# nk4517/gaussian-splatting-skysphere

Hardware: AMD Instinct MI355X
Metric: train iters/sec (fwd+bwd) + render Mpix/s @1080p, 1M Gaussians SH=3 (higher is better)
Workload: dtype f32; 1 GPU; C3: 1M Gaussians SH3 1920x1080, 16x16 tiles; gaussians=1000000, sh_degree=3, width=1920, height=1080, render_exp2=hardware v_exp_f32, parallelism=view-parallel dp1

## Files before the change

gaussian-splatting-skysphere_amd/csrc/gs_forward.hip:

```cpp
#include "gs_internal.h"

namespace gs {


template <int DEG>
__device__ __forceinline__ void sh_to_rgb(const float* __restrict__ sh, const float* __restrict__ rest, int M, float x,
                                          float y, float z, float* rgb, uint32_t& clamped) {
  constexpr int K = (DEG + 1) * (DEG + 1);
  float s[K * 3];
  if (rest) {
    const F3 d = *reinterpret_cast<const F3*>(sh);
    s[0] = d.a, s[1] = d.b, s[2] = d.c;
    const F3* r3 = reinterpret_cast<const F3*>(rest);
#pragma unroll
    for (int j = 0; j < K - 1; j++) {
      const F3 t = r3[j];
      s[3 + 3 * j] = t.a, s[4 + 3 * j] = t.b, s[5 + 3 * j] = t.c;
    }
  } else if (((M * 3) & 3) == 0) {
    const float4* s4 = reinterpret_cast<const float4*>(sh);
#pragma unroll
    for (int v = 0; v < (K * 3 + 3) / 4; v++) {
      float4 q = s4[v];
      if (4 * v + 0 < K * 3) s[4 * v + 0] = q.x;
// ... 124 lines not shown
    area += (uint32_t)__shfl_xor((int)area, d, 64);
    vis += (uint32_t)__shfl_xor((int)vis, d, 64);
  }
  if ((threadIdx.x & 63) == 0) {
    s_sum[threadIdx.x >> 6] = area;
    s_vis[threadIdx.x >> 6] = vis | (cm ? 0x80000000u : 0u);
  }
  lds_barrier();
  if (threadIdx.x == 0) {
    const uint32_t tot = s_sum[0] + s_sum[1] + s_sum[2] + s_sum[3];
    const uint32_t v4 = s_vis[0] | s_vis[1] | s_vis[2] | s_vis[3];
    const uint32_t nv = (s_vis[0] & 0x7FFFFFFFu) + (s_vis[1] & 0x7FFFFFFFu) + (s_vis[2] & 0x7FFFFFFFu) +
                        (s_vis[3] & 0x7FFFFFFFu);
    store_wg_totals(wg, b, nv, tot, (v4 >> 31) != 0);
  }
}

template <int DEG>
__global__ __launch_bounds__(256) void k_preprocess(GaussianArgs g, CameraArgs c, int* __restrict__ radii,
                                                    float4* __restrict__ splat, float4* __restrict__ binrec,
                                                    uint32_t* __restrict__ depth_key,
                                                    uint32_t* __restrict__ tiles, uint8_t* __restrict__ clamped,
                                                    WgTotals* __restrict__ wg) {
  const int b = (int)blockIdx.x + g.blk0, i = b * 256 + (int)threadIdx.x;
  uint32_t area = 0, dbits = 0;
  bool culled = false;
  if (i < g.P) {
    area = preprocess_one<DEG>(i, g, c, radii, splat, binrec, dbits, tiles, clamped, culled);
    depth_key[i] = area ? dbits : DEPTH_DROP;
  }
  workgroup_totals(area, culled, wg, (uint32_t)b);
}

template <int DEG>
__global__ __launch_bounds__(256) void k_preprocess_split(
    GaussianArgs g, CameraArgs c, int* __restrict__ radii, float4* __restrict__ splat, float4* __restrict__ binrec,
    uint32_t* __restrict__ depth_key, uint32_t* __restrict__ tiles, uint8_t* __restrict__ clamped,
    WgTotals* __restrict__ wg) {
  const int b = (int)blockIdx.x + g.blk0, i = b * 256 + (int)threadIdx.x;
  uint32_t area = 0, dbits = 0;
  bool culled = false;
  if (i < g.P) {
    area = preprocess_one<DEG, true>(i, g, c, radii, splat, binrec, dbits, tiles, clamped, culled);
    depth_key[i] = area ? dbits : DEPTH_DROP;
  }
  workgroup_totals(area, culled, wg, (uint32_t)b);
}

template <class Launch>
static void launch_row_chunks(const GaussianArgs& g, hipStream_t st, Launch&& launch) {
  const int nb = (g.P + 255) / 256;
  RowWait w[GS_MAX_ROW_WAITS];
  const int n = take_row_waits(w, GS_MAX_ROW_WAITS);
  int b0 = 0;
  for (int k = 0; k < n && b0 < nb; k++) {
    if (w[k].ev && !stream_wait(st, w[k].ev)) return;
    const int b1 = w[k].hi >= g.P ? nb : w[k].hi / 256;
    if (b1 > b0) {
      GaussianArgs gc = g;
      gc.blk0 = b0;
      launch(gc, dim3(b1 - b0));
      b0 = b1;
    }
  }
  if (b0 < nb) {
    GaussianArgs gc = g;
    gc.blk0 = b0;
    launch(gc, dim3(nb - b0));
  }
}

void fwd_preprocess(const GaussianArgs& g0, const CameraArgs& c, int* radii, const GeomPtrs& geo, hipStream_t st) {
  launch_row_chunks(g0, st, [&](const GaussianArgs& g, dim3 grid) { fwd_preprocess_grid(g, c, radii, geo, st, grid); });
}

void fwd_preprocess_grid(const GaussianArgs& g, const CameraArgs& c, int* radii, const GeomPtrs& geo, hipStream_t st,
                         dim3 grid) {
  const dim3 block(256);
  if (g.colors) {
    GS_LAUNCH("preprocess", k_preprocess<-1>, grid, block, 0, st, g, c, radii, geo.splat, geo.binrec, geo.keys_a, geo.tiles,
              geo.clamped, geo.wg_tot);
    return;
  }
  if (g.shs_rest) {
#define GS_PRE_SPLIT(D)                                                                                        \
  GS_LAUNCH("preprocess", (k_preprocess_split<D>), grid, block, 0, st, g, c, radii, geo.splat, geo.binrec, \
            geo.keys_a, geo.tiles, geo.clamped, geo.wg_tot)
    switch (g.D) {
      case 0: GS_PRE_SPLIT(0); break;
      case 1: GS_PRE_SPLIT(1); break;
      case 2: GS_PRE_SPLIT(2); break;
      default: GS_PRE_SPLIT(3); break;
    }
#undef GS_PRE_SPLIT
    return;
  }
  switch (g.D) {
    case 0:
      GS_LAUNCH("preprocess", k_preprocess<0>, grid, block, 0, st, g, c, radii, geo.splat, geo.binrec, geo.keys_a, geo.tiles,
                geo.clamped, geo.wg_tot);
      break;
    case 1:
      GS_LAUNCH("preprocess", k_preprocess<1>, grid, block, 0, st, g, c, radii, geo.splat, geo.binrec, geo.keys_a, geo.tiles,
                geo.clamped, geo.wg_tot);
      break;
    case 2:
      GS_LAUNCH("preprocess", k_preprocess<2>, grid, block, 0, st, g, c, radii, geo.splat, geo.binrec, geo.keys_a, geo.tiles,
                geo.clamped, geo.wg_tot);
      break;
    default:
      GS_LAUNCH("preprocess", k_preprocess<3>, grid, block, 0, st, g, c, radii, geo.splat, geo.binrec, geo.keys_a, geo.tiles,
                geo.clamped, geo.wg_tot);
      break;
  }
}

template <int DEG>
__global__ __launch_bounds__(256) void k_preprocess_views(GaussianArgs g, PreViews pv) {
  const int b = (int)blockIdx.x + g.blk0, i = b * 256 + (int)threadIdx.x;
  for (int v = 0; v < pv.K; v++) {
    const GeomPtrs& geo = pv.geo[v];
    uint32_t area = 0, dbits = 0;
    bool culled = false;
    if (i < g.P) {
      area = preprocess_one<DEG>(i, g, pv.c[v], pv.radii[v], geo.splat, geo.binrec, dbits, geo.tiles, geo.clamped,
                                 culled);
      geo.keys_a[i] = area ? dbits : DEPTH_DROP;
    }
    workgroup_totals(area, culled, geo.wg_tot, (uint32_t)b);
    lds_barrier();
  }
}

void fwd_preprocess_views(const GaussianArgs& g0, const PreViews& pv, hipStream_t st) {
  launch_row_chunks(g0, st, [&](const GaussianArgs& g, dim3 grid) {
    const dim3 block(256);
    if (g.colors) {
      GS_LAUNCH("preprocess_views", k_preprocess_views<-1>, grid, block, 0, st, g, pv);
      return;
    }
    switch (g.D) {
      case 0: GS_LAUNCH("preprocess_views", k_preprocess_views<0>, grid, block, 0, st, g, pv); break;
      case 1: GS_LAUNCH("preprocess_views", k_preprocess_views<1>, grid, block, 0, st, g, pv); break;
      case 2: GS_LAUNCH("preprocess_views", k_preprocess_views<2>, grid, block, 0, st, g, pv); break;
      default: GS_LAUNCH("preprocess_views", k_preprocess_views<3>, grid, block, 0, st, g, pv); break;
    }
  });
}


struct SrcTilesByRank {
  const uint32_t *tiles, *sorted_gid;
  uint32_t P;
  __device__ uint32_t operator()(uint32_t s) const {
    const uint32_t g = sorted_gid[s];
    return g < P ? tiles[g] : 0u;
  }
};

struct DstOffsets {
  uint32_t* offsets;
  uint32_t* first;
  const uint32_t* counters;
  uint32_t P;
  __device__ void operator()(uint32_t s, uint32_t ex, uint32_t v) const {
    offsets[s] = ex;
    const uint32_t I = counters[CNT_NREND];
    if (!dup_balanced(I, P)) return;
    for (uint32_t m = (ex + DUP_SLOTS - 1) / DUP_SLOTS; m * DUP_SLOTS < ex + v && m * DUP_SLOTS < I; m++) first[m] = s;
  }
};

constexpr uint32_t GS_TILE_SORT_BLOCKS = 4096, GS_DEPTH_SORT_BLOCKS = 4096;
struct CounterFinalize {
  static constexpr bool active = true;
  const WgTotals* wg;
  uint32_t nwg;
  uint32_t* counters;
  uint32_t* host;
  uint32_t* sticky;
  uint64_t vstride;
  uint32_t cap[FUSED_MAX_VIEWS];
  __device__ void operator()(uint32_t v) const {
    const WgTotals* wg = vptr(this->wg, vstride);
    uint32_t* counters = vptr(this->counters, vstride);
    uint32_t* host = this->host ? this->host + 8 * v : nullptr;
    const uint32_t cap = this->cap[v];
    __shared__ uint32_t s_lo[4], s_hi[4], s_v[4], s_e[4];
    unsigned long long si = 0;
    uint32_t sv = 0, se = 0;
    for (uint32_t k = threadIdx.x; k < nwg; k += SORT_THREADS) {
      const WgTotals t = wg[k];
      si += t.inst;
      sv += t.vis & 0x7FFFFFFFu;
      se |= t.vis >> 31;
    }
    uint32_t lo = (uint32_t)si, hi = (uint32_t)(si >> 32);
#pragma unroll
    for (int d = 32; d >= 1; d >>= 1) {
      const uint32_t olo = (uint32_t)__shfl_xor((int)lo, d, 64), ohi = (uint32_t)__shfl_xor((int)hi, d, 64);
      const unsigned long long a = ((unsigned long long)hi << 32 | lo) + ((unsigned long long)ohi << 32 | olo);
      lo = (uint32_t)a;
      hi = (uint32_t)(a >> 32);
      sv += (uint32_t)__shfl_xor((int)sv, d, 64);
      se |= (uint32_t)__shfl_xor((int)se, d, 64);
    }
    const uint32_t w = threadIdx.x >> 6;
    if ((threadIdx.x & 63) == 0) s_lo[w] = lo, s_hi[w] = hi, s_v[w] = sv, s_e[w] = se;
    lds_barrier();
    if (threadIdx.x == 0) {
      unsigned long long I = 0;
      uint32_t V = 0, e = 0;
      for (int k = 0; k < SORT_THREADS / 64; k++) {
        I += (unsigned long long)s_hi[k] << 32 | s_lo[k];
        V += s_v[k];
        e |= s_e[k];
      }
      const uint32_t err = (e ? ERR_PREFILTERED : 0u) | (I > (unsigned long long)GS_MAX_INSTANCES ? ERR_INSTANCES : 0u) |
                           (I > (unsigned long long)cap ? ERR_CAPACITY : 0u);
      counters[CNT_NREND] = (uint32_t)I;
      counters[CNT_V] = V;
      counters[CNT_ERR] = err;
      counters[CNT_I] = 0u;
      counters[CNT_LB_TILE] = 0u;
      counters[CNT_SEQ] = counters[CNT_SEQ] + 1u;
      if (host) {
        host[0] = (uint32_t)I;
        host[1] = (uint32_t)(I >> 32);
        host[2] = V;
        host[3] = err;
      }
      if (sticky && err) {
        sticky[0] = err;
        sticky[1] = (uint32_t)I;
        sticky[2] = (uint32_t)(I >> 32);
      }
    }
  }
};

void fwd_scan(int P, const GeomPtrs& geo, hipStream_t st);

void fwd_order(int P, const GeomPtrs& geo, hipStream_t st, uint32_t* host_counts, hipEvent_t counts_ready,
               const uint32_t* cap, uint32_t* sticky, int views, uint64_t vstride) {
  const uint32_t n = (uint32_t)P;
  const SortPlan sp = sort_plan(n, GS_DEPTH_SORT_BLOCKS);
  CounterFinalize fin{geo.wg_tot, (n + 255) / 256, geo.counters, host_counts, sticky, vstride, {}};
  for (int v = 0; v < FUSED_MAX_VIEWS; v++) fin.cap[v] = cap && v < views ? cap[v] : 0xFFFFFFFFu;
  GS_LAUNCH("radix_hist", k_radix_hist<CounterFinalize>, dim3(sp.nb + 1, views), dim3(SORT_THREADS), 0, st,
            geo.keys_a, nullptr, n, 0, radix_first_bits(32), sp.chunk, sp.nb, geo.sort_scratch, true, vstride, fin);
  if (counts_ready) (void)hipEventRecord(counts_ready, st);
  if (lb_tiles(n) <= LB_STATIC_MAX) {
    radix_sort_pairs(geo.keys_a, geo.vals_a, geo.keys_b, geo.vals_b, true, &geo.counters[CNT_V], n, 32,
                     geo.sort_scratch, st, true, true, nullptr, nullptr, nullptr,
                     nullptr, GS_DEPTH_SORT_BLOCKS, views, vstride);
  } else {
    radix_sort_pairs(geo.keys_a, geo.vals_a, geo.keys_b, geo.vals_b, true, &geo.counters[CNT_V], n, 32,
                     geo.sort_scratch, st, true, true, geo.tiles, geo.rtiles_a,
                     geo.rtiles_b, nullptr, GS_DEPTH_SORT_BLOCKS, views, vstride);
  }
  for (int v = 0; v < views; v++) {
    GeomPtrs g = geo;
    if (v) geom_layout((size_t)P, &g, (char*)geo.splat + (uint64_t)v * vstride);
    fwd_scan(P, g, st);
  }
}

__global__ __launch_bounds__(64) void k_clear_flags(uint32_t* __restrict__ err, uint32_t bits) {
  if (threadIdx.x == 0) err[0] = err[0] & ~bits;
}
void fwd_clear_flags(const GeomPtrs& geo, uint32_t bits, hipStream_t st) {
  GS_LAUNCH("clear_flags", k_clear_flags, dim3(1), dim3(64), 0, st, &geo.counters[CNT_ERR], bits);
}

void fwd_scan(int P, const GeomPtrs& geo, hipStream_t st) {
  const uint32_t n = (uint32_t)P;
  if (lb_tiles(n) <= LB_STATIC_MAX) {
    scan_exclusive_lb(SrcTilesByRank{geo.tiles, geo.sorted_gid, n}, DstOffsets{geo.offsets, geo.dup_first, geo.counters, n},
                      &geo.counters[CNT_V], n, geo.lb_status, &geo.counters[CNT_LB_TILE], &geo.counters[CNT_I],
                      &geo.counters[CNT_ERR], st, &geo.counters[CNT_SEQ]);
  } else {
    scan_exclusive(SrcArray{geo.tiles_by_rank}, DstOffsets{geo.offsets, geo.dup_first, geo.counters, n},
                   &geo.counters[CNT_V], n, geo.scan_partial, &geo.counters[CNT_I], st);
  }
}

__device__ __forceinline__ SpanCtx span_of(const float4* __restrict__ binrec, uint32_t gid, int& y0, int& y1) {
  const float4 a = binrec[2 * gid], b = binrec[2 * gid + 1];
  const uint32_t xr = __float_as_uint(b.z), yr = __float_as_uint(b.w);
  y0 = (int)(yr & 0xFFFFu);
  y1 = (int)(yr >> 16);
  return span_ctx(a.x, a.y, a.z, a.w, b.x, b.y, (int)(xr & 0xFFFFu), (int)(xr >> 16));
}

__global__ __launch_bounds__(256) void k_duplicate(uint32_t P, const uint32_t* __restrict__ counters,
                                                   const uint32_t* __restrict__ sorted_gid,
                                                   const uint32_t* __restrict__ offsets,
                                                   const float4* __restrict__ binrec, int gx,
                                                   uint32_t* __restrict__ tile_keys,
                                                   uint32_t* __restrict__ presort_gid) {
  const uint32_t s = blockIdx.x * 256 + threadIdx.x;
  if (s >= P || s >= counters[CNT_V] || (counters[CNT_ERR] & ERR_INVALID)) return;
  const uint32_t gid = sorted_gid[s];
  uint32_t off = offsets[s];
  int y0, y1;
  const SpanCtx sp = span_of(binrec, gid, y0, y1);
  for (int ty = y0; ty < y1; ty++) {
    int ta, tb;
    row_span(sp, ty, ta, tb);
    for (int x = ta; x < tb; x++) {
      tile_keys[off] = (uint32_t)(ty * gx + x);
      presort_gid[off] = gid;
      off++;
    }
  }
}

constexpr int DUP_THREADS = 256;
constexpr int DUP_ITEMS = DUP_SLOTS / DUP_THREADS;
__device__ __forceinline__ uint32_t own_idx(uint32_t i) { return i + (i >> 3); }

__global__ __launch_bounds__(DUP_THREADS) void k_duplicate_lb(
    uint32_t I, const uint32_t* __restrict__ counters, const uint32_t* __restrict__ dup_first,
    const uint32_t* __restrict__ sorted_gid, const uint32_t* __restrict__ offsets,
    const float4* __restrict__ binrec, int gx, int gy, uint32_t* __restrict__ tile_keys,
    uint32_t* __restrict__ presort_gid, uint2* __restrict__ ranges, uint32_t* __restrict__ hist0, uint32_t mask0,
    uint32_t* __restrict__ n_copy, uint64_t gs, uint64_t bs, uint64_t is) {
  counters = vptr(counters, gs), dup_first = vptr(dup_first, gs), sorted_gid = vptr(sorted_gid, gs);
  offsets = vptr(offsets, gs), binrec = vptr(binrec, gs);
  tile_keys = vptr(tile_keys, bs), presort_gid = vptr(presort_gid, bs), hist0 = vptr(hist0, bs);
  n_copy = vptr(n_copy, bs), ranges = vptr(ranges, is);
  __shared__ uint32_t s_own[DUP_SLOTS + DUP_SLOTS / 8];
  __shared__ uint32_t s_seg_base[DUP_SLOTS];
  __shared__ uint32_t s_seg_gid[DUP_SLOTS];
  __shared__ uint32_t s_wmax[DUP_THREADS / 64];
  __shared__ uint32_t s_nseg;
  __shared__ uint32_t s_hist[RADIX];
  const uint32_t b = blockIdx.x, tid = threadIdx.x;
  s_hist[tid] = 0;
  const uint32_t tiles = (uint32_t)(gx * gy);
  for (uint32_t t = b * DUP_THREADS + tid; t < tiles; t += gridDim.x * DUP_THREADS) ranges[t] = make_uint2(0u, 0u);
  const uint32_t V = counters[CNT_V];
  I = min(I, counters[CNT_NREND]);
  if (b == 0 && tid == 0) n_copy[0] = I;
  const uint32_t k0 = b * DUP_SLOTS;
  const uint32_t k1 = k0 < I ? min(k0 + DUP_SLOTS, I) : k0;
  if (counters[CNT_ERR] & ERR_INVALID) {
    const uint32_t g0 = 0u;
    for (uint32_t k = k0 + tid; k < k1; k += DUP_THREADS) {
      tile_keys[k] = 0u;
      presort_gid[k] = g0;
    }
    if (hist0) {
      hist0[(size_t)tid * gridDim.x + b] = tid == 0 ? k1 - k0 : 0u;
    }
    return;
  }
  if (k1 == k0) {
    if (hist0) hist0[(size_t)tid * gridDim.x + b] = 0u;
    return;
  }
  const uint32_t s_lo = dup_first[b];
  const uint32_t s_hi = (k1 < I) ? dup_first[b + 1] : V - 1;
  const uint32_t nG = s_hi - s_lo + 1;
  for (uint32_t i = tid; i < DUP_SLOTS + DUP_SLOTS / 8; i += DUP_THREADS) s_own[i] = 0;
  if (tid == 0) s_nseg = 0;
  lds_barrier();
  for (uint32_t r = tid; r < nG; r += DUP_THREADS) {
    const uint32_t gid = sorted_gid[s_lo + r];
    uint32_t pos = offsets[s_lo + r];
    if (pos >= k1) continue;
    int y0, y1;
    const SpanCtx sp = span_of(binrec, gid, y0, y1);
    for (int ty = y0; ty < y1 && pos < k1; ty++) {
      int ta, tb;
      row_span(sp, ty, ta, tb);
      const uint32_t w = (uint32_t)(tb - ta);
      if (w && pos + w > k0) {
        const uint32_t seg = atomicAdd(&s_nseg, 1u);
        s_seg_base[seg] = (uint32_t)(ty * gx + ta) - pos;
        s_seg_gid[seg] = gid;
        const uint32_t at = (pos > k0 ? pos : k0) - k0;
        s_own[own_idx(at)] = ((at + 1) << 16) | seg;
      }
      pos += w;
    }
  }
  lds_barrier();
  uint32_t v[DUP_ITEMS];
  uint32_t run = 0;
#pragma unroll
  for (int r = 0; r < DUP_ITEMS; r++) {
    run = max(run, s_own[own_idx(tid * DUP_ITEMS + r)]);
    v[r] = run;
  }
  uint32_t incl = run;
  const uint32_t lane = tid & 63;
#pragma unroll
  for (int d = 1; d < 64; d <<= 1) {
    const uint32_t o = (uint32_t)__shfl_up((int)incl, d, 64);
    if (lane >= (uint32_t)d) incl = max(incl, o);
  }
  if (lane == 63) s_wmax[tid >> 6] = incl;
  uint32_t excl = (uint32_t)__shfl_up((int)incl, 1, 64);
  if (lane == 0) excl = 0;
  lds_barrier();
  for (uint32_t w = 0; w < (tid >> 6); w++) excl = max(excl, s_wmax[w]);
#pragma unroll
  for (int r = 0; r < DUP_ITEMS; r++) s_own[own_idx(tid * DUP_ITEMS + r)] = max(v[r], excl);
  lds_barrier();
#pragma unroll
  for (int r = 0; r < DUP_ITEMS; r++) {
    const uint32_t i = (uint32_t)r * DUP_THREADS + tid;
    const uint32_t k = k0 + i;
    if (k < k1) {
      const uint32_t o = s_own[own_idx(i)] & 0xFFFFu;
      const uint32_t key = s_seg_base[o] + k;
      tile_keys[k] = key;
      presort_gid[k] = s_seg_gid[o];
      if (hist0) atomicAdd(&s_hist[key & mask0], 1u);
    }
  }
  if (hist0) {
    lds_barrier();
    hist0[(size_t)tid * gridDim.x + b] = s_hist[tid];
  }
}

__global__ __launch_bounds__(256) void k_ranges(uint32_t I, const uint32_t* __restrict__ n_dev,
                                                const uint32_t* __restrict__ tile, uint2* __restrict__ ranges,
                                                uint32_t* __restrict__ sched, uint32_t n_sched, uint32_t tiles,
                                                uint64_t bs, uint64_t is) {
  n_dev = vptr(n_dev, bs), tile = vptr(tile, bs), ranges = vptr(ranges, is), sched = vptr(sched, is);
  for (uint32_t i = blockIdx.x * 256 + threadIdx.x; i < n_sched; i += gridDim.x * 256) sched[i] = 0u;
  I = min(I, *n_dev);
// ... 266 lines not shown
```

gaussian-splatting-skysphere_amd/csrc/gs_sortscan.h:

```cpp
#pragma once
#include "gs_common.h"

namespace gs {

constexpr int SCAN_THREADS = 256;
constexpr int SCAN_ITEMS = 4;
constexpr int SCAN_TILE = SCAN_THREADS * SCAN_ITEMS;
constexpr int SCAN_MAX_BLOCKS = 1024;

struct ScanPlan {
  uint32_t nb;
  uint32_t chunk;
};

inline ScanPlan scan_plan(uint64_t n_max) {
  uint64_t tiles = (n_max + SCAN_TILE - 1) / SCAN_TILE;
  if (tiles == 0) tiles = 1;
  uint64_t per = (tiles + SCAN_MAX_BLOCKS - 1) / SCAN_MAX_BLOCKS;
  ScanPlan p;
  p.nb = (uint32_t)((tiles + per - 1) / per);
  p.chunk = (uint32_t)(per * SCAN_TILE);
  return p;
}

__device__ __forceinline__ uint32_t resolve_n(const uint32_t* n_dev, uint32_t n_max) {
  if (n_dev == nullptr) return n_max;
  uint32_t n = *n_dev;
  return n < n_max ? n : n_max;
}

__device__ __forceinline__ uint32_t wave_incl_scan(uint32_t v) {
  const uint32_t lane = __lane_id();
#pragma unroll
  for (int d = 1; d < 64; d <<= 1) {
    uint32_t t = __shfl_up(v, d, 64);
    if (lane >= (uint32_t)d) v += t;
  }
  return v;
}

__device__ __forceinline__ uint32_t block_excl_scan(uint32_t v, uint32_t* sh, uint32_t* total) {
  const uint32_t lane = __lane_id(), wid = threadIdx.x >> 6;
  uint32_t inc = wave_incl_scan(v);
  if (lane == 63) sh[wid] = inc;
  lds_barrier();
  uint32_t w0 = sh[0], w1 = sh[1], w2 = sh[2], w3 = sh[3];
  uint32_t before = (wid > 0 ? w0 : 0) + (wid > 1 ? w1 : 0) + (wid > 2 ? w2 : 0);
  *total = w0 + w1 + w2 + w3;
  lds_barrier();
  return before + inc - v;
}

template <class Src>
__global__ __launch_bounds__(SCAN_THREADS) void k_scan_reduce(Src src, const uint32_t* n_dev, uint32_t n_max,
                                                              uint32_t chunk, uint32_t* partial) {
  __shared__ uint32_t sh[4];
  const uint32_t n = resolve_n(n_dev, n_max);
  const uint64_t start = (uint64_t)blockIdx.x * chunk;
  const uint64_t end = start + chunk < n ? start + chunk : n;
  uint32_t s = 0;
  for (uint64_t i = start + threadIdx.x; i < end; i += SCAN_THREADS) s += src((uint32_t)i);
  uint32_t tot;
  block_excl_scan(s, sh, &tot);
  if (threadIdx.x == 0) partial[blockIdx.x] = tot;
}

template <int = 0>
__global__ __launch_bounds__(1024) void k_scan_partials(uint32_t* partial, uint32_t nb, uint32_t* total_out) {
  __shared__ uint32_t sh[16];
  const uint32_t lane = __lane_id(), wid = threadIdx.x >> 6;
  uint32_t carry = 0;
  for (uint32_t base = 0; base < nb; base += 1024) {
    uint32_t i = base + threadIdx.x;
    uint32_t v = i < nb ? partial[i] : 0u;
    uint32_t inc = wave_incl_scan(v);
    if (lane == 63) sh[wid] = inc;
    lds_barrier();
    uint32_t before = 0, tot = 0;
    for (uint32_t w = 0; w < 16; w++) {
      uint32_t x = sh[w];
      if (w < wid) before += x;
      tot += x;
    }
    if (i < nb) partial[i] = carry + before + inc - v;
    carry += tot;
    lds_barrier();
  }
  if (threadIdx.x == 0 && total_out) *total_out = carry;
}

template <class Src, class Dst>
__global__ __launch_bounds__(SCAN_THREADS) void k_scan_down(Src src, Dst dst, const uint32_t* n_dev,
                                                            uint32_t n_max, uint32_t chunk,
                                                            const uint32_t* partial) {
  __shared__ uint32_t sh[4];
  const uint32_t n = resolve_n(n_dev, n_max);
  const uint64_t start = (uint64_t)blockIdx.x * chunk;
  const uint64_t end = start + chunk < n ? start + chunk : n;
  uint32_t carry = partial[blockIdx.x];
  for (uint64_t base = start; base < end; base += SCAN_TILE) {
    uint64_t i0 = base + (uint64_t)threadIdx.x * SCAN_ITEMS;
    uint32_t v[SCAN_ITEMS], loc = 0;
#pragma unroll
    for (int k = 0; k < SCAN_ITEMS; k++) {
      v[k] = (i0 + k < end) ? src((uint32_t)(i0 + k)) : 0u;
      loc += v[k];
    }
    uint32_t tot;
    uint32_t ex = block_excl_scan(loc, sh, &tot) + carry;
#pragma unroll
    for (int k = 0; k < SCAN_ITEMS; k++) {
      if (i0 + k < end) dst((uint32_t)(i0 + k), ex, v[k]);
      ex += v[k];
    }
    carry += tot;
  }
}

template <class Src, class Dst>
inline void scan_exclusive(Src src, Dst dst, const uint32_t* n_dev, uint32_t n_max, uint32_t* partial,
                           uint32_t* total_out, hipStream_t st) {
  ScanPlan p = scan_plan(n_max);
  GS_LAUNCH("scan_reduce", (k_scan_reduce<Src>), dim3(p.nb), dim3(SCAN_THREADS), 0, st, src, n_dev, n_max,
            p.chunk, partial);
  GS_LAUNCH("scan_partials", k_scan_partials<>, dim3(1), dim3(1024), 0, st, partial, p.nb, total_out);
  GS_LAUNCH("scan_down", (k_scan_down<Src, Dst>), dim3(p.nb), dim3(SCAN_THREADS), 0, st, src, dst, n_dev, n_max,
            p.chunk, partial);
}

constexpr int LB_THREADS = 256;
constexpr int LB_ITEMS = 8;
constexpr int LB_TILE = LB_THREADS * LB_ITEMS;
constexpr uint64_t LB_AGG = 1, LB_PREFIX = 2;
constexpr uint32_t LB_SPIN_LIMIT = 1u << 22;
constexpr uint32_t LB_STATIC_MAX = 512;

inline uint32_t lb_tiles(uint64_t n_max) { return (uint32_t)((n_max + LB_TILE - 1) / LB_TILE) + (n_max == 0); }

__device__ __forceinline__ uint64_t lb_word(uint32_t epoch, uint64_t state, uint32_t v) {
  return ((uint64_t)epoch << 34) | (state << 32) | v;
}
__device__ __forceinline__ void lb_store(uint64_t* p, uint64_t w) {
  __hip_atomic_store(p, w, __ATOMIC_RELAXED, __HIP_MEMORY_SCOPE_AGENT);
}
__device__ __forceinline__ uint64_t lb_load(const uint64_t* p) {
  return __hip_atomic_load(p, __ATOMIC_RELAXED, __HIP_MEMORY_SCOPE_AGENT);
}

template <class Src, class Dst>
__global__ __launch_bounds__(LB_THREADS) void k_scan_lb(Src src, Dst dst, const uint32_t* n_dev, uint32_t n_max,
                                                        uint64_t* __restrict__ status, uint32_t* tile_counter,
                                                        uint32_t epoch, const uint32_t* epoch_seq,
                                                        uint32_t* total_out, uint32_t* err_flag,
                                                        uint32_t spin_limit) {
  if (epoch_seq) epoch = ((epoch + *epoch_seq) % ((1u << 30) - 1u)) + 1u;
  __shared__ uint32_t sh[4];
  __shared__ uint32_t s_tile, s_excl;
  uint32_t tile = blockIdx.x;
  if (gridDim.x > LB_STATIC_MAX) {
    if (threadIdx.x == 0) s_tile = atomicAdd(tile_counter, 1u);
    lds_barrier();
    tile = s_tile;
  }
  const uint32_t n = resolve_n(n_dev, n_max);
  const uint64_t i0 = (uint64_t)tile * LB_TILE + (uint64_t)threadIdx.x * LB_ITEMS;
  uint32_t v[LB_ITEMS], loc = 0;
#pragma unroll
  for (int k = 0; k < LB_ITEMS; k++) {
    v[k] = (i0 + k < n) ? src((uint32_t)(i0 + k)) : 0u;
    loc += v[k];
  }
  uint32_t agg;
  uint32_t ex = block_excl_scan(loc, sh, &agg);
  if (threadIdx.x < 64) {
    const uint32_t lane = threadIdx.x;
    if (lane == 0) lb_store(&status[tile], lb_word(epoch, tile == 0 ? LB_PREFIX : LB_AGG, agg));
    uint32_t excl = 0;
    int64_t t = (int64_t)tile - 1;
    while (t >= 0) {
      uint64_t w[4];
      bool ready = true;
#pragma unroll
      for (int k = 0; k < 4; k++) {
        const int64_t idx = t - 4 * (int64_t)lane - k;
        w[k] = idx >= 0 ? lb_load(&status[idx]) : lb_word(epoch, LB_PREFIX, 0);
        ready = ready && (uint32_t)(w[k] >> 34) == epoch;
      }
      uint32_t spins = 0;
      bool forced = spin_limit == 0;
      while (forced || __ballot(!ready) != 0) {
        __builtin_amdgcn_s_sleep(1);
        ready = true;
#pragma unroll
        for (int k = 0; k < 4; k++) {
          const int64_t idx = t - 4 * (int64_t)lane - k;
          if ((uint32_t)(w[k] >> 34) != epoch) w[k] = lb_load(&status[idx]);
          ready = ready && (uint32_t)(w[k] >> 34) == epoch;
        }
        if (forced || ++spins > spin_limit) {
          if (lane == 0) atomicOr(err_flag, 4u);
#pragma unroll
          for (int k = 0; k < 4; k++) w[k] = lb_word(epoch, LB_PREFIX, 0);
          ready = true;
          forced = false;
        }
      }
      int kf = 4;
#pragma unroll
      for (int k = 3; k >= 0; k--)
        if (((w[k] >> 32) & 3u) == LB_PREFIX) kf = k;
      const uint64_t pm = __ballot(kf < 4);
      const uint32_t stop = pm ? (uint32_t)__builtin_ctzll(pm) : 64u;
      uint32_t c = 0;
#pragma unroll
      for (int k = 0; k < 4; k++)
        if (lane < stop || (lane == stop && k <= kf)) c += (uint32_t)w[k];
#pragma unroll
      for (int d = 32; d >= 1; d >>= 1) c += (uint32_t)__shfl_xor((int)c, d, 64);
      excl += c;
      if (pm) break;
      t -= 256;
    }
    if (lane == 0) {
      if (tile > 0) lb_store(&status[tile], lb_word(epoch, LB_PREFIX, excl + agg));
      s_excl = excl;
      if (tile == gridDim.x - 1 && total_out) *total_out = excl + agg;
    }
  }
  lds_barrier();
  ex += s_excl;
#pragma unroll
  for (int k = 0; k < LB_ITEMS; k++) {
    if (i0 + k < n) dst((uint32_t)(i0 + k), ex, v[k]);
    ex += v[k];
  }
}

uint32_t next_scan_epoch();
uint32_t scan_spin_limit();

template <class Src, class Dst>
inline void scan_exclusive_lb(Src src, Dst dst, const uint32_t* n_dev, uint32_t n_max, uint64_t* status,
                              uint32_t* tile_counter, uint32_t* total_out, uint32_t* err_flag, hipStream_t st,
                              const uint32_t* epoch_seq, const char* name = "scan_lb") {
  const uint32_t tiles = lb_tiles(n_max);
  GS_LAUNCH(name, (k_scan_lb<Src, Dst>), dim3(tiles), dim3(LB_THREADS), 0, st, src, dst, n_dev, n_max, status,
            tile_counter, next_scan_epoch(), epoch_seq, total_out, err_flag, scan_spin_limit());
}

struct SrcArray {
  const uint32_t* a;
  __device__ uint32_t operator()(uint32_t i) const { return a[i]; }
};
struct DstArray {
  uint32_t* a;
  __device__ void operator()(uint32_t i, uint32_t ex, uint32_t) const { a[i] = ex; }
};

constexpr uint32_t DEPTH_DROP = 0xFFFFFFFFu;
constexpr int RADIX_BITS = 8;
constexpr int RADIX = 1 << RADIX_BITS;
constexpr int SORT_THREADS = 256;
constexpr int SORT_ITEMS = 8;
constexpr int SORT_TILE = SORT_THREADS * SORT_ITEMS;
constexpr int SORT_MAX_BLOCKS = 4096;

struct SortPlan {
  uint32_t nb, chunk;
};

inline int radix_passes(int end_bit) { return (end_bit + RADIX_BITS - 1) / RADIX_BITS; }
inline int radix_width(int end_bit) {
  const int np = radix_passes(end_bit);
  return (end_bit + np - 1) / np;
}
inline int radix_first_bits(int end_bit) {
  const int w = radix_width(end_bit);
  if (end_bit <= w) return end_bit;
  return end_bit - (radix_passes(end_bit) - 1) * w;
}

inline SortPlan sort_plan(uint64_t n_max, uint32_t max_blocks = SORT_MAX_BLOCKS) {
  uint64_t tiles = (n_max + SORT_TILE - 1) / SORT_TILE;
  if (tiles == 0) tiles = 1;
  if (max_blocks == 0 || max_blocks > SORT_MAX_BLOCKS) max_blocks = SORT_MAX_BLOCKS;
  uint64_t per = (tiles + max_blocks - 1) / max_blocks;
  SortPlan p;
  p.nb = (uint32_t)((tiles + per - 1) / per);
  p.chunk = (uint32_t)(per * SORT_TILE);
  return p;
}

inline size_t sort_scratch_words(uint64_t n_max) {
  uint64_t tiles = (n_max + SORT_TILE - 1) / SORT_TILE;
  if (tiles == 0) tiles = 1;
  const size_t nb = (size_t)(tiles < SORT_MAX_BLOCKS ? tiles : SORT_MAX_BLOCKS);
  return (size_t)RADIX * nb + RADIX + 16;
}

template <class T>
__device__ __forceinline__ T* vptr(T* p, uint64_t vstride) {
  return p ? (T*)((char*)p + (uint64_t)blockIdx.y * vstride) : p;
}
template <class T>
__device__ __forceinline__ const T* vptr(const T* p, uint64_t vstride) {
  return p ? (const T*)((const char*)p + (uint64_t)blockIdx.y * vstride) : p;
}

__device__ __forceinline__ uint64_t digit_peers(uint32_t d, bool valid, int bits) {
  uint64_t peers = __ballot(valid);
#pragma unroll
  for (int b = 0; b < bits; b++) {
    const uint64_t bb = __ballot((d >> b) & 1);
    peers &= ((d >> b) & 1) ? bb : ~bb;
  }
  return peers;
}

struct NoFin {
  static constexpr bool active = false;
  __device__ void operator()(uint32_t) const {}
};
__device__ __forceinline__ void radix_row_scan(uint32_t* row, uint32_t nb, uint32_t* row_total, uint32_t* sh) {
  uint32_t carry = 0;
  for (uint32_t base = 0; base < nb; base += SORT_THREADS * 4) {
    const uint32_t i0 = base + threadIdx.x * 4;
    uint32_t v[4], loc = 0;
#pragma unroll
    for (int k = 0; k < 4; k++) {
      v[k] = i0 + k < nb ? row[i0 + k] : 0u;
      loc += v[k];
    }
    uint32_t tot;
    uint32_t ex = block_excl_scan(loc, sh, &tot) + carry;
#pragma unroll
    for (int k = 0; k < 4; k++) {
      if (i0 + k < nb) row[i0 + k] = ex;
      ex += v[k];
    }
    carry += tot;
  }
  if (threadIdx.x == 0) *row_total = carry;
}

template <class Fin = NoFin>
__global__ __launch_bounds__(SORT_THREADS) void k_radix_hist(const uint32_t* __restrict__ keys, const uint32_t* n_dev,
                                                             uint32_t n_max, int shift, int bits, uint32_t chunk,
                                                             uint32_t nb, uint32_t* __restrict__ hist, bool drop,
                                                             uint64_t vstride, Fin fin = Fin()) {
  __shared__ uint32_t h[RADIX];
  if constexpr (Fin::active) {
    if (blockIdx.x == nb) {
      fin(blockIdx.y);
      return;
    }
  }
  keys = vptr(keys, vstride), n_dev = vptr(n_dev, vstride), hist = vptr(hist, vstride);
  const uint32_t n = resolve_n(n_dev, n_max);
  h[threadIdx.x] = 0;
  lds_barrier();
  const uint64_t start = (uint64_t)blockIdx.x * chunk;
  const uint64_t end = start + chunk < n ? start + chunk : n;
  const uint32_t mask = (1u << bits) - 1u;
  for (uint64_t t0 = start; t0 < end; t0 += SORT_TILE) {
    uint32_t d[SORT_ITEMS];
    bool v[SORT_ITEMS];
#pragma unroll
    for (int k = 0; k < SORT_ITEMS; k++) {
      const uint64_t i = t0 + (uint64_t)k * SORT_THREADS + threadIdx.x;
      const uint32_t key = i < end ? keys[i] : DEPTH_DROP;
      v[k] = i < end && !(drop && key == DEPTH_DROP);
      d[k] = (key >> shift) & mask;
    }
#pragma unroll
    for (int k = 0; k < SORT_ITEMS; k++)
      if (v[k]) atomicAdd(&h[d[k]], 1u);
  }
  lds_barrier();
  hist[(size_t)threadIdx.x * nb + blockIdx.x] = h[threadIdx.x];
}

template <int = 0>
__global__ __launch_bounds__(SORT_THREADS) void k_radix_rowscan(uint32_t* __restrict__ hist, uint32_t nb,
                                                                        uint32_t* __restrict__ row_total,
                                                                        uint64_t vstride) {
  __shared__ uint32_t sh[4];
  hist = vptr(hist, vstride), row_total = vptr(row_total, vstride);
  radix_row_scan(hist + (size_t)blockIdx.x * nb, nb, row_total + blockIdx.x, sh);
}

template <bool AUX, int BITS>
__global__ __launch_bounds__(SORT_THREADS) void k_radix_scatter(
    const uint32_t* __restrict__ keys_in, const uint32_t* __restrict__ vals_in, uint32_t* __restrict__ keys_out,
    uint32_t* __restrict__ vals_out, const uint32_t* n_dev, uint32_t n_max, int shift, uint32_t chunk,
    uint32_t nb, const uint32_t* __restrict__ hist, const uint32_t* __restrict__ row_total, bool drop,
    const uint32_t* __restrict__ aux_in, uint32_t* __restrict__ aux_out, uint64_t vstride) {
  __shared__ uint32_t s_base[RADIX];
  __shared__ uint32_t s_wcnt[4][RADIX];
  __shared__ uint32_t s_loc[RADIX];
  __shared__ uint32_t s_tot[RADIX];
  __shared__ uint32_t s_scan[4];
  __shared__ uint32_t s_key[SORT_TILE];
  __shared__ uint32_t s_val[SORT_TILE];
  __shared__ uint32_t s_aux[AUX ? SORT_TILE : 1];
  keys_in = vptr(keys_in, vstride), vals_in = vptr(vals_in, vstride), keys_out = vptr(keys_out, vstride);
  vals_out = vptr(vals_out, vstride), n_dev = vptr(n_dev, vstride), hist = vptr(hist, vstride);
  row_total = vptr(row_total, vstride), aux_in = vptr(aux_in, vstride), aux_out = vptr(aux_out, vstride);
  const uint32_t n = resolve_n(n_dev, n_max);
  const uint32_t tid = threadIdx.x, wid = tid >> 6, lane = tid & 63;
  {
    uint32_t all;
    const uint32_t digit_base = block_excl_scan(row_total[tid], s_scan, &all);
    s_base[tid] = digit_base + hist[(size_t)tid * nb + blockIdx.x];
  }
  const uint32_t start = blockIdx.x * chunk;
  const uint32_t end = start + chunk < n ? start + chunk : n;
  constexpr uint32_t mask = (1u << BITS) - 1u;
  for (uint32_t t0 = start; t0 < end; t0 += SORT_TILE) {
    s_wcnt[0][tid] = 0;
    s_wcnt[1][tid] = 0;
    s_wcnt[2][tid] = 0;
    s_wcnt[3][tid] = 0;
    lds_barrier();
    uint32_t key[SORT_ITEMS], val[SORT_ITEMS], rank[SORT_ITEMS], aux[AUX ? SORT_ITEMS : 1];
#pragma unroll
    for (int r = 0; r < SORT_ITEMS; r++) {
      const uint32_t i = t0 + wid * (SORT_ITEMS * 64) + (uint32_t)r * 64 + lane;
      const bool v = i < end;
      key[r] = v ? keys_in[i] : 0xFFFFFFFFu;
      val[r] = v ? (vals_in ? vals_in[i] : (uint32_t)i) : 0u;
      if constexpr (AUX) aux[r] = v ? aux_in[i] : 0u;
    }
#pragma unroll
    for (int r = 0; r < SORT_ITEMS; r++) {
      const uint32_t i = t0 + wid * (SORT_ITEMS * 64) + (uint32_t)r * 64 + lane;
      const bool v = i < end && !(drop && key[r] == DEPTH_DROP);
      const uint32_t d = (key[r] >> shift) & mask;
      const uint64_t peers = digit_peers(d, v, BITS);
      const uint32_t before = (uint32_t)__popcll(peers & lanemask_lt());
      const uint32_t run = v ? s_wcnt[wid][d] : 0u;
      rank[r] = run + before;
      __builtin_amdgcn_wave_barrier();
      if (v && before == 0) s_wcnt[wid][d] = run + (uint32_t)__popcll(peers);
      __builtin_amdgcn_wave_barrier();
    }
    lds_barrier();
    const uint32_t c0 = s_wcnt[0][tid], c1 = s_wcnt[1][tid], c2 = s_wcnt[2][tid], c3 = s_wcnt[3][tid];
    const uint32_t tot = c0 + c1 + c2 + c3;
    uint32_t tot_all;
    const uint32_t loc = block_excl_scan(tot, s_scan, &tot_all);
    s_wcnt[0][tid] = 0;
    s_wcnt[1][tid] = c0;
    s_wcnt[2][tid] = c0 + c1;
    s_wcnt[3][tid] = c0 + c1 + c2;
    s_loc[tid] = loc;
    s_tot[tid] = tot;
    lds_barrier();
#pragma unroll
    for (int r = 0; r < SORT_ITEMS; r++) {
// ... 105 lines not shown
```

Before: 1211 iters/s.

## Batch decoupled-lookback scan across views and batch gather loads

The lookback scan kernel now takes a view dimension in its grid, so multiple views are scanned in one launch instead of one launch per view. Tiles can be coarsened (SUB items per block) to stay within the static tile limit. The tile-count source now issues all index loads before the dependent gathers to raise memory-level parallelism. The render-count read in the destination functor is hoisted out of the per-element call. With dp1 and a single view, the multi-view path likely does not run, so only the load batching and the hoisted read apply.

```diff
diff --git a/gaussian-splatting-skysphere_amd/csrc/gs_forward.hip b/gaussian-splatting-skysphere_amd/csrc/gs_forward.hip
--- a/gaussian-splatting-skysphere_amd/csrc/gs_forward.hip
+++ b/gaussian-splatting-skysphere_amd/csrc/gs_forward.hip
@@ -300,9 +300,18 @@
 struct SrcTilesByRank {
   const uint32_t *tiles, *sorted_gid;
   uint32_t P;
-  __device__ uint32_t operator()(uint32_t s) const {
-    const uint32_t g = sorted_gid[s];
-    return g < P ? tiles[g] : 0u;
+  template <int N>
+  __device__ void load(uint64_t s0, uint32_t n, uint32_t* v) const {
+    uint32_t g[N];
+#pragma unroll
+    for (int k = 0; k < N; k++) g[k] = sorted_gid[s0 + k < n ? s0 + k : 0];
+#pragma unroll
+    for (int k = 0; k < N; k++) v[k] = tiles[g[k] < P ? g[k] : 0u];
+#pragma unroll
+    for (int k = 0; k < N; k++) v[k] = (s0 + k < n && g[k] < P) ? v[k] : 0u;
+  }
+  __device__ SrcTilesByRank at_offset(uint64_t off) const {
+    return SrcTilesByRank{at_bytes(tiles, off), at_bytes(sorted_gid, off), P};
   }
 };
 
@@ -311,11 +320,15 @@
   uint32_t* first;
   const uint32_t* counters;
   uint32_t P;
+  uint32_t I;
   __device__ void operator()(uint32_t s, uint32_t ex, uint32_t v) const {
     offsets[s] = ex;
-    const uint32_t I = counters[CNT_NREND];
     if (!dup_balanced(I, P)) return;
     for (uint32_t m = (ex + DUP_SLOTS - 1) / DUP_SLOTS; m * DUP_SLOTS < ex + v && m * DUP_SLOTS < I; m++) first[m] = s;
+  }
+  __device__ DstOffsets at_offset(uint64_t off) const {
+    const uint32_t* c = at_bytes(counters, off);
+    return DstOffsets{at_bytes(offsets, off), at_bytes(first, off), c, P, c[CNT_NREND]};
   }
 };
 
@@ -387,7 +400,7 @@
   }
 };
 
-void fwd_scan(int P, const GeomPtrs& geo, hipStream_t st);
+void fwd_scan(int P, const GeomPtrs& geo, hipStream_t st, int views = 1, uint64_t vstride = 0);
 
 void fwd_order(int P, const GeomPtrs& geo, hipStream_t st, uint32_t* host_counts, hipEvent_t counts_ready,
                const uint32_t* cap, uint32_t* sticky, int views, uint64_t vstride) {
@@ -407,6 +420,10 @@
                      geo.sort_scratch, st, true, true, geo.tiles, geo.rtiles_a,
                      geo.rtiles_b, nullptr, GS_DEPTH_SORT_BLOCKS, views, vstride);
   }
+  if (views > 1 && lb_tiles(n) <= LB_STATIC_MAX) {
+    fwd_scan(P, geo, st, views, vstride);
+    return;
+  }
   for (int v = 0; v < views; v++) {
     GeomPtrs g = geo;
     if (v) geom_layout((size_t)P, &g, (char*)geo.splat + (uint64_t)v * vstride);
@@ -421,14 +438,14 @@
   GS_LAUNCH("clear_flags", k_clear_flags, dim3(1), dim3(64), 0, st, &geo.counters[CNT_ERR], bits);
 }
 
-void fwd_scan(int P, const GeomPtrs& geo, hipStream_t st) {
+void fwd_scan(int P, const GeomPtrs& geo, hipStream_t st, int views, uint64_t vstride) {
   const uint32_t n = (uint32_t)P;
   if (lb_tiles(n) <= LB_STATIC_MAX) {
-    scan_exclusive_lb(SrcTilesByRank{geo.tiles, geo.sorted_gid, n}, DstOffsets{geo.offsets, geo.dup_first, geo.counters, n},
+    scan_exclusive_lb(SrcTilesByRank{geo.tiles, geo.sorted_gid, n}, DstOffsets{geo.offsets, geo.dup_first, geo.counters, n, 0u},
                       &geo.counters[CNT_V], n, geo.lb_status, &geo.counters[CNT_LB_TILE], &geo.counters[CNT_I],
-                      &geo.counters[CNT_ERR], st, &geo.counters[CNT_SEQ]);
+                      &geo.counters[CNT_ERR], st, &geo.counters[CNT_SEQ], "scan_lb", views, vstride);
   } else {
-    scan_exclusive(SrcArray{geo.tiles_by_rank}, DstOffsets{geo.offsets, geo.dup_first, geo.counters, n},
+    scan_exclusive(SrcArray{geo.tiles_by_rank}, DstOffsets{geo.offsets, geo.dup_first, geo.counters, n, 0u},
                    &geo.counters[CNT_V], n, geo.scan_partial, &geo.counters[CNT_I], st);
   }
 }
diff --git a/gaussian-splatting-skysphere_amd/csrc/gs_sortscan.h b/gaussian-splatting-skysphere_amd/csrc/gs_sortscan.h
--- a/gaussian-splatting-skysphere_amd/csrc/gs_sortscan.h
+++ b/gaussian-splatting-skysphere_amd/csrc/gs_sortscan.h
@@ -94,6 +94,7 @@
                                                             uint32_t n_max, uint32_t chunk,
                                                             const uint32_t* partial) {
   __shared__ uint32_t sh[4];
+  dst = dst.at_offset(0);
   const uint32_t n = resolve_n(n_dev, n_max);
   const uint64_t start = (uint64_t)blockIdx.x * chunk;
   const uint64_t end = start + chunk < n ? start + chunk : n;
@@ -128,6 +129,24 @@
             p.chunk, partial);
 }
 
+template <class T>
+__device__ __forceinline__ T* vptr(T* p, uint64_t vstride) {
+  return p ? (T*)((char*)p + (uint64_t)blockIdx.y * vstride) : p;
+}
+template <class T>
+__device__ __forceinline__ const T* vptr(const T* p, uint64_t vstride) {
+  return p ? (const T*)((const char*)p + (uint64_t)blockIdx.y * vstride) : p;
+}
+
+template <class T>
+__host__ __device__ __forceinline__ T* at_bytes(T* p, uint64_t bytes) {
+  return p ? (T*)((char*)p + bytes) : p;
+}
+template <class T>
+__host__ __device__ __forceinline__ const T* at_bytes(const T* p, uint64_t bytes) {
+  return p ? (const T*)((const char*)p + bytes) : p;
+}
+
 constexpr int LB_THREADS = 256;
 constexpr int LB_ITEMS = 8;
 constexpr int LB_TILE = LB_THREADS * LB_ITEMS;
@@ -147,31 +166,38 @@
   return __hip_atomic_load(p, __ATOMIC_RELAXED, __HIP_MEMORY_SCOPE_AGENT);
 }
 
-template <class Src, class Dst>
+template <class Src, class Dst, int SUB = 1>
 __global__ __launch_bounds__(LB_THREADS) void k_scan_lb(Src src, Dst dst, const uint32_t* n_dev, uint32_t n_max,
                                                         uint64_t* __restrict__ status, uint32_t* tile_counter,
                                                         uint32_t epoch, const uint32_t* epoch_seq,
                                                         uint32_t* total_out, uint32_t* err_flag,
-                                                        uint32_t spin_limit) {
+                                                        uint32_t spin_limit, uint32_t view0, uint64_t vstride) {
+  const uint64_t voff = (uint64_t)(view0 + blockIdx.y) * vstride;
+  src = src.at_offset(voff), dst = dst.at_offset(voff);
+  n_dev = at_bytes(n_dev, voff), status = at_bytes(status, voff), tile_counter = at_bytes(tile_counter, voff);
+  epoch_seq = at_bytes(epoch_seq, voff), total_out = at_bytes(total_out, voff), err_flag = at_bytes(err_flag, voff);
   if (epoch_seq) epoch = ((epoch + *epoch_seq) % ((1u << 30) - 1u)) + 1u;
   __shared__ uint32_t sh[4];
   __shared__ uint32_t s_tile, s_excl;
   uint32_t tile = blockIdx.x;
-  if (gridDim.x > LB_STATIC_MAX) {
+  if (gridDim.x * gridDim.y > LB_STATIC_MAX) {
     if (threadIdx.x == 0) s_tile = atomicAdd(tile_counter, 1u);
     lds_barrier();
     tile = s_tile;
   }
   const uint32_t n = resolve_n(n_dev, n_max);
-  const uint64_t i0 = (uint64_t)tile * LB_TILE + (uint64_t)threadIdx.x * LB_ITEMS;
-  uint32_t v[LB_ITEMS], loc = 0;
-#pragma unroll
-  for (int k = 0; k < LB_ITEMS; k++) {
-    v[k] = (i0 + k < n) ? src((uint32_t)(i0 + k)) : 0u;
-    loc += v[k];
-  }
-  uint32_t agg;
-  uint32_t ex = block_excl_scan(loc, sh, &agg);
+  const uint64_t i0 = (uint64_t)tile * SUB * LB_TILE + (uint64_t)threadIdx.x * LB_ITEMS;
+  uint32_t v[SUB][LB_ITEMS], ex[SUB], agg = 0;
+#pragma unroll
+  for (int j = 0; j < SUB; j++) src.template load<LB_ITEMS>(i0 + (uint64_t)j * LB_TILE, n, v[j]);
+#pragma unroll
+  for (int j = 0; j < SUB; j++) {
+    uint32_t loc = 0, tot;
+#pragma unroll
+    for (int k = 0; k < LB_ITEMS; k++) loc += v[j][k];
+    ex[j] = block_excl_scan(loc, sh, &tot) + agg;
+    agg += tot;
+  }
   if (threadIdx.x < 64) {
     const uint32_t lane = threadIdx.x;
     if (lane == 0) lb_store(&status[tile], lb_word(epoch, tile == 0 ? LB_PREFIX : LB_AGG, agg));
@@ -228,33 +254,69 @@
     }
   }
   lds_barrier();
-  ex += s_excl;
-#pragma unroll
-  for (int k = 0; k < LB_ITEMS; k++) {
-    if (i0 + k < n) dst((uint32_t)(i0 + k), ex, v[k]);
-    ex += v[k];
+  const uint32_t excl = s_excl;
+#pragma unroll
+  for (int j = 0; j < SUB; j++) {
+    uint32_t e = ex[j] + excl;
+#pragma unroll
+    for (int k = 0; k < LB_ITEMS; k++) {
+      const uint64_t i = i0 + (uint64_t)j * LB_TILE + k;
+      if (i < n) dst((uint32_t)i, e, v[j][k]);
+      e += v[j][k];
+    }
   }
 }
 
 uint32_t next_scan_epoch();
 uint32_t scan_spin_limit();
 
+constexpr int LB_MAX_SUB = 4;
+inline int lb_sub(uint32_t tiles, int views) {
+  int sub = 1;
+  while (sub < LB_MAX_SUB && views > 1 && (uint64_t)((tiles + sub - 1) / sub) * (uint64_t)views > LB_STATIC_MAX)
+    sub *= 2;
+  return sub;
+}
 template <class Src, class Dst>
 inline void scan_exclusive_lb(Src src, Dst dst, const uint32_t* n_dev, uint32_t n_max, uint64_t* status,
                               uint32_t* tile_counter, uint32_t* total_out, uint32_t* err_flag, hipStream_t st,
-                              const uint32_t* epoch_seq, const char* name = "scan_lb") {
+                              const uint32_t* epoch_seq, const char* name = "scan_lb", int views = 1,
+                              uint64_t vstride = 0) {
   const uint32_t tiles = lb_tiles(n_max);
-  GS_LAUNCH(name, (k_scan_lb<Src, Dst>), dim3(tiles), dim3(LB_THREADS), 0, st, src, dst, n_dev, n_max, status,
-            tile_counter, next_scan_epoch(), epoch_seq, total_out, err_flag, scan_spin_limit());
+  const uint32_t spin = scan_spin_limit();
+  const int sub = lb_sub(tiles, views);
+  const uint32_t gx = (tiles + sub - 1) / sub;
+  const uint32_t per = gx < LB_STATIC_MAX ? LB_STATIC_MAX / gx : 1u;
+#define GS_SCAN_LB(SUB)                                                                                           \
+  GS_LAUNCH(name, (k_scan_lb<Src, Dst, SUB>), dim3(gx, nv), dim3(LB_THREADS), 0, st, src, dst, n_dev, n_max, status, \
+            tile_counter, next_scan_epoch(), epoch_seq, total_out, err_flag, spin, v0, vstride)
+  for (uint32_t v0 = 0; v0 < (uint32_t)views; v0 += per) {
+    const uint32_t nv = (uint32_t)views - v0 < per ? (uint32_t)views - v0 : per;
+    switch (sub) {
+      case 1: GS_SCAN_LB(1); break;
+      case 2: GS_SCAN_LB(2); break;
+      default: GS_SCAN_LB(4); break;
+    }
+  }
+#undef GS_SCAN_LB
 }
 
 struct SrcArray {
   const uint32_t* a;
   __device__ uint32_t operator()(uint32_t i) const { return a[i]; }
+  template <int N>
+  __device__ void load(uint64_t i0, uint32_t n, uint32_t* v) const {
+#pragma unroll
+    for (int k = 0; k < N; k++) v[k] = a[i0 + k < n ? i0 + k : 0];
+#pragma unroll
+    for (int k = 0; k < N; k++) v[k] = i0 + k < n ? v[k] : 0u;
+  }
+  __device__ SrcArray at_offset(uint64_t off) const { return SrcArray{at_bytes(a, off)}; }
 };
 struct DstArray {
   uint32_t* a;
   __device__ void operator()(uint32_t i, uint32_t ex, uint32_t) const { a[i] = ex; }
+  __device__ DstArray at_offset(uint64_t off) const { return DstArray{at_bytes(a, off)}; }
 };
 
 constexpr uint32_t DEPTH_DROP = 0xFFFFFFFFu;
@@ -296,15 +358,6 @@
   if (tiles == 0) tiles = 1;
   const size_t nb = (size_t)(tiles < SORT_MAX_BLOCKS ? tiles : SORT_MAX_BLOCKS);
   return (size_t)RADIX * nb + RADIX + 16;
-}
-
-template <class T>
-__device__ __forceinline__ T* vptr(T* p, uint64_t vstride) {
-  return p ? (T*)((char*)p + (uint64_t)blockIdx.y * vstride) : p;
-}
-template <class T>
-__device__ __forceinline__ const T* vptr(const T* p, uint64_t vstride) {
-  return p ? (const T*)((const char*)p + (uint64_t)blockIdx.y * vstride) : p;
 }
 
 __device__ __forceinline__ uint64_t digit_peers(uint32_t d, bool valid, int bits) {
```

Result: faster. 1225 iters/s, median of 6 (+1.2%).
